# superlinear-ai/raglite

Measured on AMD Instinct MI355X. Metric: queries/sec, MaxSim 32x1M d=1024 exact top-100, higher is better.
Workload: dtype f32 in / f32 scores: candidate chunks found with the fp16 hi halves of corpus and queries (1 x v_mfma_f32_16x16x32_f16 per multiply, f32 accumulate, rigorous error bound), their scores by v_mfma_f32_16x16x4_f32 (exact f32 products); full-precision fallback: 3 x v_mfma_f32_16x16x32_f16 on hi+lo pairs

## Files before the change

### include/raglite_hip.h

```cpp
#ifndef RAGLITE_HIP_H
#define RAGLITE_HIP_H

#include <stddef.h>
#include <stdint.h>

#ifdef __cplusplus
extern "C" {
#endif

typedef enum {
    RL_OK = 0,
    RL_ERR_INVALID = -1,
    RL_ERR_HIP = -2,
    RL_ERR_UNSUPPORTED = -3,
    RL_ERR_NOMEM = -4
} rl_status;

typedef enum { RL_MEM_HOST = 0, RL_MEM_DEVICE = 1 } rl_mem;
#define RL_MEM_FILTERS_DEVICE 2
typedef enum {
    RL_ARITH_AUTO = 0,
    RL_ARITH_FP32_EXACT = 1,
    RL_ARITH_F16_SPLIT = 2,
    RL_ARITH_F16_STORED = 3
// ... 70 lines not shown
                  const float* row_sumsq, float split_scale, int32_t kernel, int32_t max_workgroups, float* out, int64_t ld,
                  float* out_q_sumsq, float* out_q_scale, int mem, void* stream);

int rl_index_create(rl_index** out, const float* embeddings, int64_t n_rows, int32_t dim,
                    const int64_t* chunk_offsets, int64_t n_chunks, int metric, int mem, void* stream);
int rl_index_create_f16(rl_index** out, const uint16_t* embeddings_f16, int64_t n_rows, int32_t dim,
                        const int64_t* chunk_offsets, int64_t n_chunks, int metric, int mem, void* stream);
int rl_index_destroy(rl_index* index);
int rl_index_info(const rl_index* index, int64_t* n_rows, int32_t* dim, int64_t* n_chunks, int* metric);
int rl_index_memory(const rl_index* index, int64_t out[8]);

#define RL_IMAGE_PRESPLIT 1u
#define RL_IMAGE_HI 2u
#define RL_IMAGE_HI_PLANE 4u
int rl_index_prepare(rl_index* index, uint32_t images, uint32_t* built, void* stream);

int rl_index_append(rl_index* index, const float* rows, int64_t n_new_rows, const int64_t* new_chunk_sizes,
                    int64_t n_new_chunks, int mem, void* stream);
int rl_index_delete_chunks(rl_index* index, const int64_t* chunk_ordinals, int64_t n, void* stream);
int rl_index_live(rl_index* index, int64_t* live_rows, int64_t* live_chunks, void* stream);
int rl_index_compact(rl_index* index, int64_t* out_remap, int64_t* new_n_rows, int64_t* new_n_chunks, void* stream);

int rl_index_set_arithmetic(rl_index* index, int mode);
int rl_index_arithmetic(rl_index* index, int* in_effect);

typedef enum {
    RL_OPT_HI_SEARCH = 1, RL_OPT_HI_MAXSIM = 2, RL_OPT_HI_PRODUCTS = 3, RL_OPT_PP_PASS = 4, RL_OPT_FUSED_TOPK = 5, RL_OPT_FUSED_HI = 6,
    RL_OPT_FUSED_PP = 7, RL_OPT_FUSED_TOPK_CAP = 8, RL_OPT_FUSED_TOPK_STRIDE = 9, RL_OPT_GEMM_PASS = 10, RL_OPT_QUERY_PAIRS = 11,
    RL_OPT_PLANES_GEMM = 12, RL_OPT_KEEP_IMAGE = 13, RL_OPT_KEEP_HI = 14, RL_OPT_IMAGE_HEADROOM_MB = 15, RL_OPT_ARITHMETIC = 16,
    RL_OPT_EXACT_KTH_THRESHOLD = 17, RL_OPT_FUSED_TWO_ROUNDS = 18, RL_OPT_KEEP_HI_PLANE = 19, RL_OPT_PAIRS_PACKED = 20,
    RL_OPT_F16_EXACT = 21, RL_OPT_LAZY_IMAGES = 22, RL_OPT_FUSED_PP_SAMPLE = 23,
    RL_OPT_LIST_SELECT = 24, RL_OPT_HI_FEW = 25, RL_OPT_TOPK_BLOCK = 26, RL_OPT_HI_PIVOT = 27, RL_OPT_COUNT_ = 28
} rl_option;
enum { RL_OPT_PP_SCHEDULE = 64, RL_OPT_PP_XCD_PASSES = 65 };
int rl_set_default_option(int key, int64_t value);
int rl_get_default_option(int key, int64_t* value);
int rl_index_set_option(rl_index* index, int key, int64_t value);
int rl_index_get_option(rl_index* index, int key, int64_t* value);

int rl_search_rows(rl_index* index, const float* queries, int32_t n_queries, int32_t k,
                   float* out_scores, int32_t* out_rows, int mem, void* stream);

int rl_rank_cut_begin(rl_index* index, const float* queries, int32_t n_queries, int mem, void* stream);
int rl_rank_cut_level(rl_index* index, int level, int64_t rank_limit, uint32_t* out_hist, int mem, void* stream);
int rl_rank_cut_level_done(rl_index* index, int level, const uint32_t* hist_sum, int mem, void* stream);
int rl_rank_cut_ties(rl_index* index, int64_t rank_limit, uint32_t* out_ties, int mem, void* stream);
int rl_rank_cut_finish(rl_index* index, int64_t rank_limit, const uint32_t* ties_before, const uint32_t* chunk_filter, int32_t k,
                       float* out_scores, int32_t* out_rows, int mem, void* stream);

int rl_search_chunks(rl_index* index, const float* queries, int32_t n_queries, int32_t num_hits,
                     int32_t k, float* out_scores, int32_t* out_chunks, int32_t* out_counts,
                     int mem, void* stream);

int rl_maxsim_topk(rl_index* index, const float* query_vecs, int32_t nq, int32_t k,
                   float* out_scores, int32_t* out_chunks, int mem, void* stream);
int rl_maxsim_scores(rl_index* index, const float* query_vecs, int32_t nq, float* out_scores,
                     int mem, void* stream);
int rl_maxsim_topk_batch(rl_index* index, const float* query_vecs, int32_t n_queries, int32_t nq, int32_t k,
                         float* out_scores, int32_t* out_chunks, int mem, void* stream);
int rl_maxsim_topk_batch_f16(rl_index* index, const uint16_t* query_vecs_f16, int32_t n_queries, int32_t nq, int32_t k,
                             float* out_scores, int32_t* out_chunks, int mem, void* stream);

int rl_maxsim_batch_begin(rl_index* index, const float* query_vecs, int32_t n_queries, int32_t nq, int32_t k, float* out_approx, int mem,
                          void* stream);
int rl_maxsim_batch_finish(rl_index* index, const float* query_vecs, const float* all_approx, int32_t world, int32_t rank, float* out_scores,
                           int32_t* out_chunks, int mem, void* stream);

// ... 181 lines not shown
```

### raglite_amd/_abi.py

```python

from __future__ import annotations

import ctypes as C
import functools
import os
from pathlib import Path

LIB_PATH = Path(os.environ.get("RAGLITE_HIP_LIB") or Path(__file__).resolve().parent / "_lib" / "libraglite_hip.so")

RL_OK, RL_ERR_INVALID, RL_ERR_HIP, RL_ERR_UNSUPPORTED, RL_ERR_NOMEM = 0, -1, -2, -3, -4
MEM_HOST, MEM_DEVICE = 0, 1
MEM_FILTERS_DEVICE = 2
METRICS = {"cosine": 0, "dot": 1, "l2": 2}
SCORE_METRICS = {"raw": 0, "cosine": 1, "dot": 2, "l2": 3}
SYNTH_KINDS = {"uniform": 0, "small_int": 1}
ATTN_DTYPES = {"bfloat16": 0, "float16": 1}
ENCODER_MAX_TOKENS = 256
ENCODER_MAX_PACK_TOKENS = 8192
ENCODER_EPILOGUES = {"bias": 0, "gelu": 1, "partial": 2}
OPTIONS = {
    "hi_search": 1, "hi_maxsim": 2, "hi_products": 3, "pp_pass": 4, "fused_topk": 5, "fused_hi": 6, "fused_pp": 7, "fused_topk_cap": 8,
    "fused_topk_stride": 9, "gemm_pass": 10, "query_pairs": 11, "planes_gemm": 12, "keep_image": 13, "keep_hi": 14,
    "image_headroom_mb": 15, "arithmetic": 16, "exact_kth_threshold": 17, "fused_two_rounds": 18,
    "keep_hi_plane": 19, "pairs_packed": 20, "f16_exact": 21, "lazy_images": 22, "fused_pp_sample": 23, "list_select": 24, "hi_few": 25, "topk_block": 26, "hi_pivot": 27,
}
SCHEDULE_OPTIONS = {"pp_schedule": 64, "pp_xcd_passes": 65}


def option_key(name: str) -> int:
    return OPTIONS[name] if name in OPTIONS else SCHEDULE_OPTIONS[name]

c_void_p, c_int, c_i32, c_i64, c_u64, c_size_t = C.c_void_p, C.c_int, C.c_int32, C.c_int64, C.c_uint64, C.c_size_t
c_double, c_char_p = C.c_double, C.c_char_p

_SIGNATURES = {
    "rl_version": [],
    "rl_last_error": [],
    "rl_init": [c_int],
    "rl_device_count": [C.POINTER(c_int)],
    "rl_device_info": [c_int, c_char_p, c_int, C.POINTER(c_int), C.POINTER(c_i64)],
    "rl_dev_alloc": [C.POINTER(c_void_p), c_size_t],
    "rl_dev_free": [c_void_p],
    "rl_memcpy_h2d": [c_void_p, c_void_p, c_size_t, c_void_p],
    "rl_memcpy_d2h": [c_void_p, c_void_p, c_size_t, c_void_p],
    "rl_memcpy_d2d": [c_void_p, c_void_p, c_size_t, c_void_p],
    "rl_stream_sync": [c_void_p],
    "rl_synth_fill": [c_void_p, c_i64, c_i64, c_u64, c_int, c_void_p],
    "rl_pool_norm": [c_void_p, c_i64, c_i32, c_void_p, c_void_p, c_i64, c_i32, c_double, c_void_p, c_void_p,
                     c_int, c_void_p],
    "rl_attention_varlen": [c_void_p, c_void_p, c_i32, c_i64, c_i32, c_i32, c_i32, c_i32, C.c_float, c_void_p, c_int, c_void_p],
    "rl_encoder_create": [C.POINTER(c_void_p), c_i32, c_i32, c_i32, c_i32, c_i32, c_i32, c_i32, C.c_float, c_i32, c_void_p, c_void_p, c_void_p,
                          c_void_p, c_void_p, c_void_p],
    "rl_encoder_forward": [c_void_p, c_void_p, c_void_p, c_void_p, c_void_p, c_i32, c_i64, c_i32, c_void_p, c_int, c_void_p],
    "rl_encoder_info": [c_void_p, c_i64, C.POINTER(c_i32), C.POINTER(c_i64), C.POINTER(c_i64), C.POINTER(c_void_p), C.POINTER(c_i32)],
    "rl_encoder_destroy": [c_void_p],
    "rl_encoder_embed": [c_void_p, c_void_p, c_void_p, c_i64, c_void_p, c_i32, c_void_p, c_i32, c_void_p, c_i32, c_void_p, c_void_p, c_i32,
                         C.c_float, c_i32, c_void_p, c_int, c_void_p],
    "rl_encoder_linear": [c_void_p, c_i64, c_i32, c_void_p, c_i32, c_void_p, c_i32, c_i32, c_void_p, c_void_p, c_int, c_void_p],
    "rl_encoder_layer_norm": [c_void_p, c_i32, c_i64, c_i32, c_void_p, c_void_p, c_void_p, c_void_p, C.c_float, c_i32, c_void_p, c_int,
# ... 192 lines not shown
```

### raglite_amd/csrc/api.hip

```cpp
#include <cmath>
#include <cstdlib>
#include <cstring>
#include <limits>
#include <memory>
#include <mutex>
#include <utility>
#include <vector>

#include "handles.h"

namespace rl {

static thread_local std::string g_last_error;
void set_error(const std::string& msg) { g_last_error = msg; }
int fail(int code, const std::string& msg) {
    g_last_error = msg;
    return code;
}

namespace {

int scan_mode(int metric) {
    switch (metric) {
        case RL_COSINE: return SCAN_COSINE;
        case RL_DOT: return SCAN_DOT;
        case RL_L2: return SCAN_L2;
        default: return -1;
    }
}

std::mutex g_default_opts_mu;
Options g_default_opts;
bool option_key_ok(int key) { return (key >= 1 && key < RL_OPT_COUNT_) || key == RL_OPT_PP_SCHEDULE || key == RL_OPT_PP_XCD_PASSES; }
bool option_value_ok(int key, int64_t value) {
    switch (key) {
        case RL_OPT_HI_SEARCH: case RL_OPT_HI_MAXSIM: case RL_OPT_PP_PASS: case RL_OPT_FUSED_TOPK: case RL_OPT_FUSED_HI: case RL_OPT_FUSED_PP:
        case RL_OPT_GEMM_PASS: case RL_OPT_QUERY_PAIRS: case RL_OPT_PLANES_GEMM: case RL_OPT_KEEP_IMAGE: case RL_OPT_KEEP_HI:
        case RL_OPT_EXACT_KTH_THRESHOLD: case RL_OPT_FUSED_TWO_ROUNDS: case RL_OPT_KEEP_HI_PLANE: case RL_OPT_F16_EXACT: case RL_OPT_LAZY_IMAGES: case RL_OPT_FUSED_PP_SAMPLE: case RL_OPT_LIST_SELECT: case RL_OPT_HI_FEW: case RL_OPT_HI_PIVOT:
        case RL_OPT_PP_SCHEDULE:
            return value == 0 || value == 1;
        case RL_OPT_PP_XCD_PASSES: return value == 8 || value == 4 || value == 2 || value == 1;
        case RL_OPT_TOPK_BLOCK: case RL_OPT_PAIRS_PACKED: return value >= 0 && value <= 2;
        case RL_OPT_HI_PRODUCTS: return value == 1 || value == 2;
        case RL_OPT_FUSED_TOPK_CAP: return value >= 0 && value <= MERGE_CAP;
        case RL_OPT_FUSED_TOPK_STRIDE: return value == 0 || (value >= 2 && value <= (int64_t(1) << 20));
        case RL_OPT_IMAGE_HEADROOM_MB: return value >= -1 && value <= (int64_t(1) << 30);
        case RL_OPT_ARITHMETIC: return value == RL_ARITH_AUTO || value == RL_ARITH_FP32_EXACT;
        default: return false;
    }
}

}

int64_t default_option(int key) {
    std::lock_guard<std::mutex> lock(g_default_opts_mu);
    return g_default_opts.v[key];
}

int use_scratch(rl_index* idx, hipStream_t s) {
    ++idx->scratch_epoch;
    idx->filt = {};
    idx->ws.block_route = (int)idx->opt.v[RL_OPT_TOPK_BLOCK];
    idx->replay.valid = false;
    return idx->last_stream.use(s);
}

}

namespace {
void update_split_scale(rl_index* idx) {
    idx->split_scale = 0.f;
    if (idx->E16 || !idx->E || idx->arithmetic == RL_ARITH_FP32_EXACT || idx->nonfinite) return;
// ... 1621 lines not shown
}

int rl_maxsim_topk(rl_index* idx, const float* query_vecs, int32_t nq, int32_t k, float* out_scores,
                   int32_t* out_chunks, int mem, void* stream) {
    return rl_maxsim_topk_filtered(idx, query_vecs, nq, k, nullptr, out_scores, out_chunks, mem, stream);
}

namespace {
struct HiBatch : HiBatchScratch {
    int32_t cap = 2048;
    bool one_product; float m_abs; const float* q_unscale;
    const float* qsum = nullptr;
    bool m_ready = true;
    bool exact_kth;
    const uint32_t* filter = nullptr;
    size_t lay(Carver c, int32_t n, int32_t k) { return HiBatchScratch::lay(c, n, k, cap, pivot_scratch_words(std::min<int32_t>(n, 2))); }
};
int hi_batch_approx(rl_index* idx, const float* d_q, int32_t nq, int32_t n_queries, int32_t n_gemm, int32_t k, float* sc, int64_t ld, HiBatch& hb,
                    hipStream_t s, bool flag_zeroed = false) {
    hb.one_product = idx->opt.v[RL_OPT_HI_PRODUCTS] == 1;
    hb.exact_kth = idx->opt.on(RL_OPT_EXACT_KTH_THRESHOLD);
    RL_TRY(carve(idx->hibuf, hb, n_gemm, k));
    const int32_t cap = hb.cap;
    hb.m_abs = idx->norm_stats.max_lo_norm + sum_eps(idx->dim) * idx->norm_stats.max_row_norm;
    QueryPlanes qp;
    qp.lay(Carver(idx->qplanes.p), n_queries, idx->dim);
    hb.q_unscale = qp.meta;
    hb.qsum = qp.qsum;
    if (!flag_zeroed) RL_HIP(hipMemsetAsync(hb.flag, 0, 16 * sizeof(uint32_t), s));
    (void)cap;
    const bool pp = hb.one_product && idx->dim >= 256 && idx->opt.on(RL_OPT_PP_PASS);
    if (pp)
        RL_TRY(launch_maxsim_pp(approx_image(idx), {idx->qplanes.p, n_queries, 0, n_gemm, nq}, chunks(idx), {sc, ld}, on(idx, s),
                                (int)idx->opt.v[RL_OPT_PP_SCHEDULE], (int)idx->opt.v[RL_OPT_PP_XCD_PASSES]));
    for (int32_t b = 0; !pp && b < n_gemm; b += GEMM_PASS_QUERIES) {
        const int32_t n_q = std::min<int32_t>(GEMM_PASS_QUERIES, n_gemm - b);
        RL_TRY(launch_maxsim_gemm(approx_image(idx), {idx->qplanes.p, n_queries, b, n_q, nq}, chunks(idx), {sc + (int64_t)b * ld, ld}, on(idx, s),
                                   hb.one_product,  false));
    }
    RL_TRY(mask_chunk_scores(idx, sc, n_gemm, ld, hb.filter, s));
    int st_pv = RL_ERR_UNSUPPORTED;
    if (n_gemm < 16 && idx->n_chunks > (int64_t)262144 && idx->opt.on(RL_OPT_HI_PIVOT))
        st_pv = launch_topk_pivot(sc, n_gemm, idx->n_chunks, ld, k, idx->ws, hb.ts, hb.ti, s);
    if (st_pv != RL_OK && st_pv != RL_ERR_UNSUPPORTED) return st_pv;
    if (st_pv == RL_ERR_UNSUPPORTED) RL_TRY(launch_topk(sc, n_gemm, idx->n_chunks, ld, k, idx->ws, hb.ts, hb.ti, s));
    return RL_OK;
}
int hi_batch_fallback(rl_index* idx, const float* d_q, int32_t nq, int32_t n_queries, int32_t n_gemm, int32_t k, float* sc, int64_t ld,
                      const HiBatch& hb, float* d_s, int32_t* d_c, hipStream_t s, bool rows_only = false);
int hi_batch_rescore(rl_index* idx, const float* d_q, int32_t nq, int32_t n_queries, int32_t n_gemm, int32_t k, float* sc, int64_t ld,
                     const HiBatch& hb, float* d_s, int32_t* d_c, hipStream_t s, bool rows_only = false) {
    const QueryVecs q{d_q, nq, (int64_t)nq * idx->dim, n_gemm};
    idx->filt = {RL_FILTER_MAXSIM_BATCH, n_gemm, hb.cap, hb.cnt, hb.flag};
    const int packed = (int)idx->opt.v[RL_OPT_PAIRS_PACKED];
    const bool m_from_qsum = !hb.m_ready && hb.qsum != nullptr;
    if (!hb.m_ready && !(hb.exact_kth && k <= hb.cap && hb.qsum)) return fail(RL_ERR_INVALID, "MaxSim batch: no bound for the candidate threshold");
    if (hb.exact_kth && k <= hb.cap) {
        RL_TRY(launch_maxsim_pairs(rows(idx), q, chunks(idx), {hb.ti, k, 0, 0, packed}, hb.es_top, s));
        if (m_from_qsum)
            RL_TRY(launch_exact_threshold(hb.es_top, hb.ti, n_gemm, k, hb.m, hb.cap, hb.thr, hb.cnt, hb.ci, hb.es, hb.flag, s, hb.qsum, hb.m_abs,
                                          idx->norm_stats.max_row_norm + idx->norm_stats.max_lo_norm, hb.one_product, hb.ts));
        else
            RL_TRY(launch_exact_threshold(hb.es_top, hb.ti, n_gemm, k, hb.m, hb.cap, hb.thr, hb.cnt, hb.ci, hb.es, hb.flag, s, nullptr, 0.f, 0.f, false, hb.ts));
        RL_TRY(launch_collect_above(sc, n_gemm, idx->n_chunks, ld, hb.thr, nullptr, hb.cap, hb.ci, nullptr, hb.cnt, hb.flag, s, hb.ts, hb.ti, k));
        if (hb.cap > k)
            RL_TRY(launch_maxsim_pairs(rows(idx), q, chunks(idx), {hb.ci, hb.cap - k, hb.cap, k, packed}, hb.es, s));
    } else {
// ... 287 lines not shown
    if (idx->live_chunk_bits) RL_TRY(launch_fix_masked(d_s, d_c, (int64_t)n_queries * k, s));
    return st.finish();
}

int rl_maxsim_approx_scores(rl_index* idx, const float* query_vecs, int32_t n_queries, int32_t nq, int kernel, float* out_scores,
                            float* out_bound, int mem, void* stream) {
    if (!idx) return fail(RL_ERR_INVALID, "rl_maxsim_approx_scores: null index");
    if (n_queries < 0 || nq < 1 || (kernel != 0 && kernel != 1)) return fail(RL_ERR_INVALID, "rl_maxsim_approx_scores: bad arguments");
    if (n_queries == 0) return RL_OK;
    if (!query_vecs || !out_scores) return fail(RL_ERR_INVALID, "rl_maxsim_approx_scores: null argument");
    hipStream_t s = as_stream(stream);
    std::lock_guard<std::mutex> lock(idx->mu);
    RL_TRY(use_scratch(idx, s));
    if (idx->has_empty_chunk || idx->n_chunks == 0)
        return fail(RL_ERR_UNSUPPORTED, "rl_maxsim_approx_scores: the approximate pass needs an index without empty chunks");
    RL_TRY(demand_images(idx, approx_image_bit(idx), s));
    if (!approx_image_valid(idx) || nq > 32 || (kernel == 0 && idx->dim < 256))
        return fail(RL_ERR_UNSUPPORTED, "rl_maxsim_approx_scores: this index keeps no HI image (or nq > 32 / dim < 256)");
    Staging st(mem, s);
    const float* d_q; float* d_o; float* d_b = nullptr;
    const size_t q_elems = (size_t)nq * idx->dim;
    const int64_t ld = idx->n_chunks;
    RL_TRY(st.in(query_vecs, (size_t)n_queries * q_elems, &d_q));
    RL_TRY(st.out(out_scores, (size_t)n_queries * ld, &d_o));
    RL_TRY(st.out(out_bound, (size_t)n_queries, &d_b));
    RL_TRY(idx->qplanes.reserve(query_planes_bytes(idx->dim, n_queries)));
    RL_TRY(launch_query_planes({d_q, nq, (int64_t)q_elems, n_queries}, idx->dim, idx->qplanes.p, s, nullptr, 0));
    const int32_t per = kernel == 0 ? n_queries : GEMM_PASS_QUERIES;
    for (int32_t b = 0; b < n_queries; b += per) {
        const QueryImageRef q{idx->qplanes.p, n_queries, b, std::min<int32_t>(per, n_queries - b), nq};
        const Scores out{d_o + (int64_t)b * ld, ld};
        if (kernel == 0)
            RL_TRY(launch_maxsim_pp(approx_image(idx), q, chunks(idx), out, on(idx, s), (int)idx->opt.v[RL_OPT_PP_SCHEDULE],
                                    (int)idx->opt.v[RL_OPT_PP_XCD_PASSES]));
        else
            RL_TRY(launch_maxsim_gemm(approx_image(idx), q, chunks(idx), out, on(idx, s),  true,  false));
    }
    if (d_b) {
        const float m_abs = idx->norm_stats.max_lo_norm + sum_eps(idx->dim) * idx->norm_stats.max_row_norm;
        QueryPlanes qp;
        qp.lay(Carver(idx->qplanes.p), n_queries, idx->dim);
        const float* q_unscale = qp.meta;
        ApproxBound L;
        RL_TRY(carve(idx->hibuf, L, n_queries));
        float *const top = L.top, *const thr = L.thr;
        uint32_t *const cnt = L.cnt, *const flag = L.flag;
        RL_HIP(hipMemsetAsync(top, 0, (size_t)n_queries * sizeof(float), s));
        RL_HIP(hipMemsetAsync(flag, 0, 16 * sizeof(uint32_t), s));
        RL_TRY(launch_maxsim_threshold(top, n_queries, 1, d_q, nq, idx->dim, (int64_t)q_elems, 1.0f, m_abs, thr, cnt, flag, s, q_unscale,
                                       idx->norm_stats.max_row_norm + idx->norm_stats.max_lo_norm));
        RL_TRY(launch_scale_f32(thr, d_b, -0.5f, n_queries, s));
        idx->filt = {};
    }
    return st.finish();
}

}

namespace rl {
int maxsim_rerank_device(rl_index* idx, const float* d_q, int32_t n_queries, int32_t nq, const int32_t* d_c, int32_t n_cand, float* d_o,
                         hipStream_t s) {
    {
        const int64_t n_items = (int64_t)n_queries * n_cand;
        RL_TRY(idx->cand.reserve((size_t)n_items * sizeof(int32_t)));
        RL_TRY(launch_sanitize_candidates(d_c, n_items, idx->n_chunks, idx->live_chunk_bits, idx->cand.as<int32_t>(), s));
        d_c = idx->cand.as<int32_t>();
    }
// ... 165 lines not shown
    else if (kind == 0 || kind == 2 || kind == 3 || kind == 5 || kind == 6) {}
    else if (kind == 9) RL_TRY(idx->scores.reserve((size_t)(idx->n_cu > 0 ? idx->n_cu : 256) * 512 * sizeof(float)));
    else if (kind == 8) {
        const auto& r = idx->replay;
        if (!r.valid || r.pools[0] != idx->misc.p || r.pools[1] != idx->fused.p || r.pools[2] != idx->pp_work.p || !hi_image_valid(idx))
            return fail(RL_ERR_UNSUPPORTED, "rl_time_kernel kind 8: no fused-HI row search ran on this index since its scratch was last resized");
    }
    else RL_TRY(idx->scores.reserve(std::max<size_t>((size_t)nq * ld * sizeof(float), 16)));
    hipEvent_t e0, e1;
    RL_HIP(hipEventCreate(&e0));
    RL_HIP(hipEventCreate(&e1));
    int st = RL_OK;
    if (kind == 2) {
        st = pairs_prepare(idx, q_dev, nq / 2, (int64_t)(nq / 2) * idx->dim, 2, s);
        if (st != RL_OK) { (void)hipEventDestroy(e0); (void)hipEventDestroy(e1); return st == RL_ERR_UNSUPPORTED ? fail(st, "rl_time_kernel: the pair kernel does not apply to this index / shape") : st; }
    }
    if (kind == 3 || kind == 5 || kind == 6) {
        st = gemm_prepare(idx, q_dev, nq / GEMM_PASS_QUERIES, (int64_t)(nq / GEMM_PASS_QUERIES) * idx->dim, GEMM_PASS_QUERIES, s, true);
        if (st == RL_OK && !image_valid(idx)) st = RL_ERR_UNSUPPORTED;
        if (st != RL_OK) { (void)hipEventDestroy(e0); (void)hipEventDestroy(e1); return st == RL_ERR_UNSUPPORTED ? fail(st, "rl_time_kernel: the eight-query kernel does not apply to this index / shape") : st; }
    }
    if (kind == 7) {
        st = pp_vec >= 1 && pp_vec * pp_n == nq ? gemm_prepare(idx, q_dev, pp_vec, (int64_t)pp_vec * idx->dim, pp_n, s) : RL_ERR_UNSUPPORTED;
        if (st == RL_OK && !(approx_image_valid(idx) && idx->dim >= 256)) st = RL_ERR_UNSUPPORTED;
        if (st != RL_OK) { (void)hipEventDestroy(e0); (void)hipEventDestroy(e1); return st == RL_ERR_UNSUPPORTED ? fail(st, "rl_time_kernel: the sixteen-query kernel does not apply to this index / shape") : st; }
    }
    if (kind == 4 || kind == 10) {
        st = demand_images(idx, IMG_HI_PLANE, s);
        if (st != RL_OK) { (void)hipEventDestroy(e0); (void)hipEventDestroy(e1); return st; }
    }
    RL_HIP(hipEventRecord(e0, s));
    for (int i = 0; i < iters && st == RL_OK; ++i) {
        if (kind == 7) st = launch_maxsim_pp(approx_image(idx), {idx->qplanes.p, pp_n, 0, pp_n, pp_vec}, chunks(idx), {idx->scores.as<float>(), ldc}, on(idx, s),
                                             (int)idx->opt.v[RL_OPT_PP_SCHEDULE], (int)idx->opt.v[RL_OPT_PP_XCD_PASSES]);
        else if (kind == 3) st = gemm_pass(idx, nq / GEMM_PASS_QUERIES, GEMM_PASS_QUERIES, 0, GEMM_PASS_QUERIES, idx->scores.as<float>(), ldc, s);
        else if (kind == 8) {
            const auto& r = idx->replay;
            const RowMetric metric = metric_of(idx, r.mode);
            if (hipMemsetAsync(r.cnt, 0, (size_t)r.B * sizeof(uint32_t), s) != hipSuccess) st = RL_ERR_HIP;
            else if (r.pp && r.round1_tiles > 0) {
                CandArgs ca1 = r.ca;
                ca1.tau = r.thr1;
                st = launch_pp_rows_pass(hi_image(idx), r.B, r.qs, metric, &ca1, {idx->pp_work.p, r.log_cap, 0, r.round1_tiles, false, r.row_test}, on(idx, s));
                if (st == RL_OK)
                    st = launch_pp_rows_pass(hi_image(idx), r.B, r.qs, metric, &r.ca, {idx->pp_work.p, r.log_cap, r.round1_tiles, -1, true, r.row_test}, on(idx, s));
            }
            else if (r.pp) st = launch_pp_rows_pass(hi_image(idx), r.B, r.qs, metric, &r.ca, {idx->pp_work.p, r.log_cap, 0, -1, false, r.row_test}, on(idx, s));
            else st = launch_score_planes_pass(hi_image(idx), r.B, r.qs, Scores{}, metric, {1, &r.ca, true}, on(idx, s));
        }
        else if (kind == 0) st = maxsim_scores_device(idx, q_dev, nq, idx->scores.as<float>(), s);
        else if (kind == 9) st = launch_mfma_f16_rate(idx->scores.as<float>(), idx->n_cu, MFMA_RATE_ITERS, s, nullptr);
        else if (kind == 2) st = pairs_pass(idx, nq / 2, 2, 0, idx->scores.as<float>(), ldc, s);
        else if (kind == 5 || kind == 6) {
            st = hi_image_valid(idx) ? launch_maxsim_gemm(hi_image(idx), {idx->qplanes.p, GEMM_PASS_QUERIES, 0, GEMM_PASS_QUERIES, nq / GEMM_PASS_QUERIES},
                                                          chunks(idx), {idx->scores.as<float>(), ldc}, on(idx, s),  kind == 6,  false)
                                     : fail(RL_ERR_UNSUPPORTED, "rl_time_kernel: the index has no HI image");
        }
        else if (kind == 4) {
            st = hi_valid(idx) ? launch_maxsim_stream(hi_plane(idx), {q_dev, nq}, chunks(idx), 1, {idx->scores.as<float>(), ld}, on(idx, s))
                               : fail(RL_ERR_UNSUPPORTED, "rl_time_kernel: the index has no HI plane");
        }
        else if (kind == 10) {
            st = hi_valid(idx) && nq <= 32 ? launch_maxsim_stream_batch(hi_plane(idx), {q_dev, nq, (int64_t)nq * idx->dim, 1}, chunks(idx),
                                                                        {idx->scores.as<float>(), ldc}, on(idx, s))
                                           : fail(RL_ERR_UNSUPPORTED, "rl_time_kernel: the index has no HI plane (or nq > 32)");
        }
        else st = score_rows(idx, q_dev, nq, ld, s);
// ... 13 lines not shown
```

### raglite_amd/csrc/common.h

```cpp
#pragma once
#include <hip/hip_runtime.h>
#include <stdint.h>

#include <algorithm>
#include <cstdlib>
#include <string>

#include "raglite_hip.h"

namespace rl {

void set_error(const std::string& msg);
int fail(int code, const std::string& msg);

#define RL_HIP(expr)                                                                         \
    do {                                                                                     \
        hipError_t _e = (expr);                                                              \
        if (_e != hipSuccess)                                                                \
            return ::rl::fail(_e == hipErrorOutOfMemory ? RL_ERR_NOMEM : RL_ERR_HIP,         \
                              std::string(#expr) + ": " + hipGetErrorString(_e));            \
    } while (0)

#define RL_TRY(expr)              \
    do {                          \
// ... 406 lines not shown
struct Launch {
    int n_cu = 0;
    hipStream_t s = nullptr;
    const uint32_t* run_if = nullptr;
};

int launch_row_to_chunk(const int64_t* chunk_offsets, int64_t n_chunks, int64_t n_rows, int32_t* row_to_chunk,
                        hipStream_t s);
int launch_maxsim_stream(const RowsRef& D, const QueryVecs& q, const ChunkMap& c, int mode, Scores out, const Launch& on);
struct StreamSecondJob {
    const float* D = nullptr;
    int64_t n_rows = 0;
    float* out = nullptr;
    int64_t ld = 0;
    const uint32_t* run_if = nullptr;
};
int launch_maxsim_stream_two(const RowsRef& D, const QueryVecs& q, const ChunkMap& c, Scores out, const Launch& on, const StreamSecondJob& job2);
int launch_maxsim_stream_batch(const RowsRef& D, const QueryVecs& q, const ChunkMap& c, Scores out, const Launch& on);
size_t query_split_bytes(int32_t dim, int32_t n_queries);
int launch_query_split(const QueryVecs& q, int32_t dim, void* buf, bool f16_corpus, hipStream_t s);
int launch_maxsim_stream2(const RowsRef& D, const QueryImageRef& q, const ChunkMap& c, Scores out, const Launch& on);
size_t planes_bytes(int64_t rows, int32_t dim, bool half = false);
int launch_presplit_rows(const RowsRef& E, int64_t first_row, void* planes, hipStream_t s);
int launch_preformat_rows16(const RowsRef& E, int64_t first_row, void* planes, hipStream_t s);
int launch_presplit_hi_rows(const RowsRef& E, int64_t first_row, void* planes, hipStream_t s);
size_t chunk_ends_words(int64_t rows);
int launch_chunk_ends(const int32_t* row_to_chunk, int64_t n_rows, uint32_t* ends, hipStream_t s);
size_t query_planes_bytes(int32_t dim, int32_t n_queries);
int launch_query_planes(const QueryVecs& q, int32_t dim, void* buf, hipStream_t s, uint32_t* zero_words, int n_zero);
int launch_maxsim_gemm(const RowsRef& image, const QueryImageRef& q, const ChunkMap& c, Scores out, const Launch& on, bool hi_only,
                       bool all_passes);
constexpr int32_t PP_PASS_QUERIES = 16;
int launch_maxsim_pp(const RowsRef& image, const QueryImageRef& q, const ChunkMap& c, Scores out, const Launch& on,
                     int schedule, int xcd_passes);
constexpr int32_t MFMA_RATE_ITERS = 1000;
int launch_mfma_f16_rate(float* out, int n_cu, int32_t iters, hipStream_t s, double* flops);
size_t score_planes_scratch_floats(int32_t nb, int32_t dim);
int launch_score_planes(const RowsRef& image, const float* Q, int32_t nb, Scores out, const RowMetric& m, float* scratch, const Launch& on);
struct CandArgs { const float* tau; int32_t tau_stride; float* scores; int32_t* ids; uint32_t* cnt; uint32_t* overflow; int32_t cap; };
int launch_score_planes_queries(const float* Q, int32_t nb, int32_t dim, float* scratch, int mode, hipStream_t s, uint32_t* zero_word = nullptr);
size_t pp_rows_scratch_bytes(int64_t n_rows, int32_t nb, int n_cu, int32_t expected_per_query, int32_t* log_cap_out);
struct PpRowsPass {
    void* work = nullptr;
    int32_t log_cap = 0;
    int64_t tile_begin = 0, tile_count = -1;
    bool norms_ready = false;
    bool row_norm_test = false;
};
int launch_pp_rows_pass(const RowsRef& image, int32_t nb, float* scratch, const RowMetric& m, const CandArgs* cand, const PpRowsPass& pass,
                        const Launch& on);
int launch_pp_rows_sample(const RowsRef& image, int32_t nb, float* scratch, const RowMetric& m, Scores S, int32_t stride, const Launch& on);
int launch_raise_threshold(float* thr, const float* kth, int32_t nq, int32_t k, const float* window, hipStream_t s);
struct ScorePass {
    int32_t tile_stride = 1;
    const CandArgs* cand = nullptr;
    bool hi_only = false;
};
int launch_score_planes_pass(const RowsRef& image, int32_t nb, float* scratch, Scores out, const RowMetric& m, const ScorePass& pass,
                             const Launch& on);
int launch_row_range(const float* E, int64_t n_rows, int32_t dim, uint32_t* range, hipStream_t s);
int launch_score_gemm(const RowsRef& E, const float* Q, int32_t nb, Scores out, const RowMetric& m, float* q_sumsq_scratch, const Launch& on,
                      int tile = 0);
int launch_query_sumsq(const float* Q, int32_t nb, int32_t dim, float* out, hipStream_t s);
size_t score_gemm_scratch_floats(int32_t nb, int32_t dim, bool split);
struct PairsList {
    const int32_t* candidates = nullptr;
    int64_t n_items = 0;
// ... 14 lines not shown
```

### raglite_amd/csrc/handles.h

```cpp
#pragma once
#include <limits>
#include <memory>
#include <mutex>
#include <vector>

#include "device_mem.h"

namespace rl {

inline int filters_mem(int mem) { return (mem & RL_MEM_FILTERS_DEVICE) ? RL_MEM_DEVICE : mem; }
inline int args_mem(int mem) { return mem & ~RL_MEM_FILTERS_DEVICE; }

constexpr size_t SCORE_BATCH_BYTES = size_t(8) << 30;

struct Options {
    int64_t v[RL_OPT_PP_XCD_PASSES + 1];
    Options() {
        for (auto& x : v) x = 0;
        v[RL_OPT_HI_SEARCH] = v[RL_OPT_HI_MAXSIM] = v[RL_OPT_HI_PRODUCTS] = v[RL_OPT_PP_PASS] = v[RL_OPT_FUSED_TOPK] = v[RL_OPT_FUSED_HI] = 1;
        v[RL_OPT_FUSED_PP] = v[RL_OPT_GEMM_PASS] = v[RL_OPT_QUERY_PAIRS] = v[RL_OPT_PLANES_GEMM] = v[RL_OPT_KEEP_IMAGE] = v[RL_OPT_KEEP_HI] = 1;
        v[RL_OPT_EXACT_KTH_THRESHOLD] = v[RL_OPT_FUSED_TWO_ROUNDS] = v[RL_OPT_KEEP_HI_PLANE] = v[RL_OPT_F16_EXACT] = v[RL_OPT_LAZY_IMAGES] = v[RL_OPT_FUSED_PP_SAMPLE] = v[RL_OPT_LIST_SELECT] = v[RL_OPT_HI_FEW] = 1;
        v[RL_OPT_TOPK_BLOCK] = v[RL_OPT_PAIRS_PACKED] = 2;
        v[RL_OPT_HI_PIVOT] = 1;
        v[RL_OPT_PP_SCHEDULE] = 1;
        v[RL_OPT_PP_XCD_PASSES] = 2;
        v[RL_OPT_IMAGE_HEADROOM_MB] = -1;
        v[RL_OPT_ARITHMETIC] = RL_ARITH_AUTO;
    }
    bool on(int key) const { return v[key] != 0; }
};

struct Image {
    Pool buf;
    float scale = 0.f;
    int64_t rows = 0;
    void drop() {
        buf.release();
        scale = 0.f;
        rows = 0;
    }
    bool covers(float at, int64_t n_rows) const { return scale > 0.f && scale == at && rows == n_rows && n_rows > 0; }
};
struct NormStats {
    float max_row_norm = 0.f, max_lo_norm = 0.f, max_lo_ratio = 0.f;
    float min_row_norm = std::numeric_limits<float>::infinity();
    float max_row_norm_scale = 0.f;
    int64_t max_row_norm_rows = 0;
    void reset() { *this = NormStats(); }
    bool measured(int64_t n_rows) const { return max_row_norm_rows == n_rows && max_row_norm > 0.f; }
};

struct LastStream {
    hipStream_t stream = nullptr;
    bool set = false;
    int use(hipStream_t s) {
        if (set && stream != s) RL_HIP(hipStreamSynchronize(stream));
        stream = s;
        set = true;
// ... 148 lines not shown
```

### raglite_amd/csrc/maxsim_pp.hip

```cpp
#include <cstdio>
#include <cstdlib>
#include <utility>

#include "common.h"
#include "pp_schedule.h"
#include "scratch_layout.h"

namespace rl {

typedef float f32x4 __attribute__((ext_vector_type(4)));
typedef _Float16 h16x8 __attribute__((ext_vector_type(8)));

namespace {
constexpr int PP_RT = 128;
constexpr int PP_NBLK = PP_RT / 16;
constexpr int PP_QPP = 16;
constexpr int PP_DC = 8;
constexpr int PP_LC = 6;
constexpr int PP_CSLOT = PP_NBLK * 1024;
constexpr int PP_STAGE = 1536;
constexpr int PP_LDS = PP_DC * PP_CSLOT + 16 * PP_STAGE * 4;

__device__ __forceinline__ int64_t pp_uniform_i64(int64_t v) {
    const uint32_t lo = __builtin_amdgcn_readfirstlane((uint32_t)(uint64_t)v);
// ... 30 lines not shown
    f32x16s v;
    const float* const u = reinterpret_cast<const float*>(pp_uniform_i64(reinterpret_cast<int64_t>(p)));
    asm volatile("s_load_dwordx16 %0, %1, 0x0\n\ts_waitcnt lgkmcnt(0)" : "=s"(v) : "s"(u) : "memory");
    return v;
}
__device__ __forceinline__ h16x8 pp_h(const f32x4& v) {
    h16x8 r;
    __builtin_memcpy(&r, &v, 16);
    return r;
}
}

struct PpRows {
    const float* tau;
    const float* q_unscale;
    const float* q_sumsq;
    const float* row_norm;
    const float* blk_minmax;
    int32_t B, QT, metric;
    float* cand_scores; int32_t* cand_ids; uint32_t* cand_cnt; uint32_t* overflow; int32_t cap;
    uint2* log; int32_t log_cap;
    int32_t tile_begin, tile_count;
    float* S; int64_t ld_s; int32_t stride;
    int32_t xcd_passes, dma_hint;
};

template <int DBG, int MODE, bool ROWNORM>
__global__ __launch_bounds__(512, 2) void maxsim_pp_kernel(const char* __restrict__ planes, int64_t n_rows, int32_t nslab,
                                                           const char* __restrict__ qfrag, const float* __restrict__ qmeta, int32_t n_q,
                                                           const int32_t* __restrict__ row_to_chunk, const int64_t* __restrict__ chunk_offsets,
                                                           const uint32_t* __restrict__ ends_bits, float* __restrict__ out, int64_t out_stride,
                                                           float inv_e_scale, const uint32_t* __restrict__ run_if, PpRows rs) {
    constexpr bool ROWS = MODE == 2, SCORES = MODE == 1, GROUPS = ROWS || SCORES;
    constexpr bool TILES = MODE == 3;
    static_assert(!TILES || DBG == 0, "the timing skeletons keep the slab-counting loop");
    __shared__ __attribute__((aligned(16))) char smem[PP_LDS];
    if (run_if && __builtin_amdgcn_readfirstlane((int)*run_if) == 0) return;
    const int lane = threadIdx.x & 63;
    const int wv = wave_id();
    int64_t G = gridDim.x, b = blockIdx.x;
    int qt = (int)blockIdx.y;
    if constexpr (!GROUPS) {
        const int32_t passes = (n_q + PP_QPP - 1) / PP_QPP;
        const PpSlot m = gridDim.y > 1 ? pp_schedule((int32_t)blockIdx.x, (int32_t)blockIdx.y, (int32_t)gridDim.x, (int32_t)gridDim.y, passes)
                                       : pp_schedule_affine((int32_t)blockIdx.x, (int32_t)gridDim.x, passes, rs.xcd_passes);
        G = __builtin_amdgcn_readfirstlane(m.ranges);
        b = __builtin_amdgcn_readfirstlane(m.range);
        qt = __builtin_amdgcn_readfirstlane(m.pass);
    }
    auto boundary = [&](int64_t t) -> int64_t {
        if (t <= 0) return 0;
        if (t >= n_rows) return n_rows;
        const int32_t c = row_to_chunk[t];
        const int64_t c0 = chunk_offsets[c], c1 = chunk_offsets[c + 1];
        return c0 == t ? t : c1;
    };
    int32_t r_lo = 0, r_hi = 0, nt_rows = 0;
    if constexpr (!GROUPS) {
        r_lo = (int32_t)pp_uniform_i64(boundary((n_rows * b) / G));
        r_hi = (int32_t)pp_uniform_i64((b + 1 == G) ? n_rows : boundary((n_rows * (b + 1)) / G));
        if (r_hi <= r_lo) return;
    } else {
        const int64_t Tr = rs.tile_count;
        const int64_t t0 = (Tr * b) / G, t1 = (Tr * (b + 1)) / G;
        nt_rows = (int32_t)(t1 - t0);
        if (nt_rows <= 0) return;
        r_lo = (int32_t)((rs.tile_begin + t0) * PP_RT);
        r_hi = (int32_t)n_rows;
// ... 518 lines not shown
    auto main_loop = [&](auto LAG_) __attribute__((always_inline)) {
        if constexpr (TILES) {
            const int pairs = nslab >> 1;
            prologue_fragments();
            for (int t = 0; t < nt; ++t) {
                pp_tile_ends(t);
                slab(qA, qB, LAG_, std::true_type{});
                landed(qB);
                slab(qB, qA, LAG_, std::false_type{});
                landed(qA);
#pragma nounroll
                for (int p = 1; p < pairs; ++p) {
                    slab(qA, qB, LAG_, std::false_type{});
                    landed(qB);
                    slab(qB, qA, LAG_, std::false_type{});
                    landed(qA);
                }
                asm volatile("s_waitcnt lgkmcnt(0)" : "+s"(tile_ends) : : "memory");
                [&]<int... A>(std::integer_sequence<int, A...>) { (block_epilogue_maxsim(std::integral_constant<int, A>{}, t), ...); }
                (std::make_integer_sequence<int, PP_NBLK>{});
                if (own_cnt - own_flushed > PP_STAGE - PP_RT) flush_out();
            }
        } else {
            for (int g = 0; g < total; g += 2) {
                slab(qA, qB, LAG_, std::false_type{});
                landed(qB);
                if (g + 1 < total) {
                    slab(qB, qA, LAG_, std::false_type{});
                    landed(qA);
                }
            }
        }
    };
#undef PP_I
    if (wv < 4) main_loop(std::false_type{});
    else main_loop(std::true_type{});
    asm volatile("s_waitcnt vmcnt(0)" ::: "memory");
    dump_log();
    flush_rows();
    flush_out();
    if constexpr (DBG & 128) {
        if (n_q > 1000000) {
            f32x4 t = (f32x4){0.f, 0.f, 0.f, 0.f};
#pragma unroll
            for (int q = 0; q < 2; ++q)
#pragma unroll
                for (int qb = 0; qb < 2; ++qb)
#pragma unroll
                    for (int a = 0; a < PP_NBLK; ++a) t += acc[q][qb][a];
            out[lane] = (t[0] + t[1]) + (t[2] + t[3]);
        }
    }
}

int launch_maxsim_pp(const RowsRef& rows, const QueryImageRef& q, const ChunkMap& c, Scores o, const Launch& on, int schedule, int xcd_passes) {
    const auto [image, one_plane, n_rows, dim, split_scale] = rows;
    const auto [qbuf, n_queries, first, n_q, nq] = q;
    const auto [row_to_chunk, chunk_offsets, n_chunks, ends_bits] = c;
    const auto [out, out_stride] = o;
    const auto [n_cu, s, run_if] = on;
    if (!one_plane) return RL_ERR_UNSUPPORTED;
    if (nq < 1 || nq > 32 || n_q < 1 || n_q > PP_QPP * 4096 || n_rows < 1 || first < 0 || first + n_q > n_queries) return RL_ERR_UNSUPPORTED;
    if (dim % 32 || dim < 256 || !(split_scale > 0.f) || !image || !ends_bits) return RL_ERR_UNSUPPORTED;
    const int32_t nslab = dim / 32;
    const char* qfrag = static_cast<const char*>(qbuf) + (size_t)first * nslab * 4096;
    QueryPlanes L;
    L.lay(Carver(const_cast<void*>(qbuf)), n_queries, dim);
    const float* qmeta = L.meta + 2 * (size_t)first;
    const int64_t tiles = (n_rows + PP_RT - 1) / PP_RT;
    const int64_t gx = std::max<int64_t>(1, std::min<int64_t>(n_cu > 0 ? n_cu : 256, tiles)), passes = (n_q + PP_QPP - 1) / PP_QPP;
    const dim3 grid = schedule == 1 ? dim3((unsigned)(gx * passes)) : dim3((unsigned)gx, (unsigned)passes), blk(512);
    PpRows rs{};
    rs.xcd_passes = schedule == 1 ? xcd_passes : 8;
#define RL_PP_LAUNCH(DBG_) RL_PP_LAUNCH_MODE(DBG_, 0)
#define RL_PP_LAUNCH_MODE(DBG_, MODE_)                                                                                                     \
    hipLaunchKernelGGL((maxsim_pp_kernel<DBG_, MODE_, false>), grid, blk, 0, s, static_cast<const char*>(image), n_rows, nslab, qfrag, qmeta, n_q, row_to_chunk, \
                       chunk_offsets, ends_bits, out, out_stride, 1.0f / split_scale, run_if, rs)
#ifdef RAGLITE_EXPERIMENTS
    const int force_hint = std::getenv("RAGLITE_PP_HINT") ? std::atoi(std::getenv("RAGLITE_PP_HINT")) : -1;
    if (force_hint >= PP_HINT_NONE && force_hint <= PP_HINT_SC1) rs.dma_hint = force_hint;
    const int dbg = std::getenv("RAGLITE_PP_DBG") ? std::atoi(std::getenv("RAGLITE_PP_DBG")) : 0;
    if (dbg == 2) RL_PP_LAUNCH(2);
    else if (dbg == 128) RL_PP_LAUNCH(128);
    else if (dbg == 136) RL_PP_LAUNCH(136);
    else if (dbg == 144) RL_PP_LAUNCH(144);
    else if (dbg == 160) RL_PP_LAUNCH(160);
    else if (dbg == 184) RL_PP_LAUNCH(184);
    else if (dbg == 1 || nslab % 2) RL_PP_LAUNCH(0);
    else RL_PP_LAUNCH_MODE(0, 3);
#else
    if (nslab % 2) RL_PP_LAUNCH(0);
    else RL_PP_LAUNCH_MODE(0, 3);
#endif
#undef RL_PP_LAUNCH
#undef RL_PP_LAUNCH_MODE
    RL_HIP(hipGetLastError());
    return RL_OK;
}

__global__ __launch_bounds__(256) void block_norm_minmax_kernel(const float* __restrict__ row_norm, int64_t n_rows, int64_t n_blocks,
                                                                 float* __restrict__ out) {
    const int64_t blk = (int64_t)blockIdx.x * 256 + threadIdx.x;
    if (blk >= n_blocks) return;
    float mn = INFINITY, mx = 0.f;
    for (int i = 0; i < 16; ++i) {
        const int64_t r = blk * 16 + i;
        if (r < n_rows) { const float v = row_norm[r]; mn = fminf(mn, v); mx = fmaxf(mx, v); }
    }
    out[2 * blk] = mn;
    out[2 * blk + 1] = mx;
}

int launch_pp_rows_sample(const RowsRef& rows, int32_t nb, float* scratch, const RowMetric& m, Scores out, int32_t stride, const Launch& on) {
    const auto [image, one_plane, n_rows, dim, split_scale] = rows;
    const auto [mode, row_norm, row_sumsq] = m;
    const auto [S, ld_s] = out;
    const auto [n_cu, s, run_if] = on;
    if (!one_plane || run_if) return RL_ERR_UNSUPPORTED;
    if (nb < 1 || n_rows < 1 || dim % 32 || dim < 256 || !(split_scale > 0.f) || !image || !S || stride < 1) return RL_ERR_UNSUPPORTED;
    if (mode != SCAN_COSINE && mode != SCAN_DOT) return RL_ERR_UNSUPPORTED;
    if (mode == SCAN_COSINE && !row_norm) return RL_ERR_INVALID;
    if ((ld_s & 255) || (reinterpret_cast<uintptr_t>(S) & 15)) return RL_ERR_UNSUPPORTED;
    const int32_t nslab = dim / 32, groups = (nb + 31) / 32;
    ScoreQueries L;
// ... 130 lines not shown
```

Baseline: 18940.

## Add alternating double-buffered query-register main loop for MaxSim PP kernel

Adds a new kernel mode (MODE 4) with an alternating main loop. Two query register sets (qA/qB) are ping-ponged so the next slab's query and corpus loads are issued while MFMAs run on the current set. Explicit s_barrier, waitcnt and sched_barrier placement replaces the split-by-wave main_loop, and the tile epilogue is interleaved around barriers. A new pp_loop option, on by default, selects it, at the cost of more live registers and hand-tuned synchronisation that could stall or raise register pressure.

```diff
diff --git a/include/raglite_hip.h b/include/raglite_hip.h
--- a/include/raglite_hip.h
+++ b/include/raglite_hip.h
@@ -126,7 +126,7 @@
     RL_OPT_F16_EXACT = 21, RL_OPT_LAZY_IMAGES = 22, RL_OPT_FUSED_PP_SAMPLE = 23,
     RL_OPT_LIST_SELECT = 24, RL_OPT_HI_FEW = 25, RL_OPT_TOPK_BLOCK = 26, RL_OPT_HI_PIVOT = 27, RL_OPT_COUNT_ = 28
 } rl_option;
-enum { RL_OPT_PP_SCHEDULE = 64, RL_OPT_PP_XCD_PASSES = 65 };
+enum { RL_OPT_PP_SCHEDULE = 64, RL_OPT_PP_XCD_PASSES = 65, RL_OPT_PP_LOOP = 66 };
 int rl_set_default_option(int key, int64_t value);
 int rl_get_default_option(int key, int64_t* value);
 int rl_index_set_option(rl_index* index, int key, int64_t value);
diff --git a/raglite_amd/_abi.py b/raglite_amd/_abi.py
--- a/raglite_amd/_abi.py
+++ b/raglite_amd/_abi.py
@@ -24,7 +24,7 @@
     "image_headroom_mb": 15, "arithmetic": 16, "exact_kth_threshold": 17, "fused_two_rounds": 18,
     "keep_hi_plane": 19, "pairs_packed": 20, "f16_exact": 21, "lazy_images": 22, "fused_pp_sample": 23, "list_select": 24, "hi_few": 25, "topk_block": 26, "hi_pivot": 27,
 }
-SCHEDULE_OPTIONS = {"pp_schedule": 64, "pp_xcd_passes": 65}
+SCHEDULE_OPTIONS = {"pp_schedule": 64, "pp_xcd_passes": 65, "pp_loop": 66}
 
 
 def option_key(name: str) -> int:
diff --git a/raglite_amd/csrc/api.hip b/raglite_amd/csrc/api.hip
--- a/raglite_amd/csrc/api.hip
+++ b/raglite_amd/csrc/api.hip
@@ -31,13 +31,13 @@
 
 std::mutex g_default_opts_mu;
 Options g_default_opts;
-bool option_key_ok(int key) { return (key >= 1 && key < RL_OPT_COUNT_) || key == RL_OPT_PP_SCHEDULE || key == RL_OPT_PP_XCD_PASSES; }
+bool option_key_ok(int key) { return (key >= 1 && key < RL_OPT_COUNT_) || key == RL_OPT_PP_SCHEDULE || key == RL_OPT_PP_XCD_PASSES || key == RL_OPT_PP_LOOP; }
 bool option_value_ok(int key, int64_t value) {
     switch (key) {
         case RL_OPT_HI_SEARCH: case RL_OPT_HI_MAXSIM: case RL_OPT_PP_PASS: case RL_OPT_FUSED_TOPK: case RL_OPT_FUSED_HI: case RL_OPT_FUSED_PP:
         case RL_OPT_GEMM_PASS: case RL_OPT_QUERY_PAIRS: case RL_OPT_PLANES_GEMM: case RL_OPT_KEEP_IMAGE: case RL_OPT_KEEP_HI:
         case RL_OPT_EXACT_KTH_THRESHOLD: case RL_OPT_FUSED_TWO_ROUNDS: case RL_OPT_KEEP_HI_PLANE: case RL_OPT_F16_EXACT: case RL_OPT_LAZY_IMAGES: case RL_OPT_FUSED_PP_SAMPLE: case RL_OPT_LIST_SELECT: case RL_OPT_HI_FEW: case RL_OPT_HI_PIVOT:
-        case RL_OPT_PP_SCHEDULE:
+        case RL_OPT_PP_SCHEDULE: case RL_OPT_PP_LOOP:
             return value == 0 || value == 1;
         case RL_OPT_PP_XCD_PASSES: return value == 8 || value == 4 || value == 2 || value == 1;
         case RL_OPT_TOPK_BLOCK: case RL_OPT_PAIRS_PACKED: return value >= 0 && value <= 2;
@@ -1725,7 +1725,7 @@
     const bool pp = hb.one_product && idx->dim >= 256 && idx->opt.on(RL_OPT_PP_PASS);
     if (pp)
         RL_TRY(launch_maxsim_pp(approx_image(idx), {idx->qplanes.p, n_queries, 0, n_gemm, nq}, chunks(idx), {sc, ld}, on(idx, s),
-                                (int)idx->opt.v[RL_OPT_PP_SCHEDULE], (int)idx->opt.v[RL_OPT_PP_XCD_PASSES]));
+                                (int)idx->opt.v[RL_OPT_PP_SCHEDULE], (int)idx->opt.v[RL_OPT_PP_XCD_PASSES], (int)idx->opt.v[RL_OPT_PP_LOOP]));
     for (int32_t b = 0; !pp && b < n_gemm; b += GEMM_PASS_QUERIES) {
         const int32_t n_q = std::min<int32_t>(GEMM_PASS_QUERIES, n_gemm - b);
         RL_TRY(launch_maxsim_gemm(approx_image(idx), {idx->qplanes.p, n_queries, b, n_q, nq}, chunks(idx), {sc + (int64_t)b * ld, ld}, on(idx, s),
@@ -2079,7 +2079,7 @@
         const Scores out{d_o + (int64_t)b * ld, ld};
         if (kernel == 0)
             RL_TRY(launch_maxsim_pp(approx_image(idx), q, chunks(idx), out, on(idx, s), (int)idx->opt.v[RL_OPT_PP_SCHEDULE],
-                                    (int)idx->opt.v[RL_OPT_PP_XCD_PASSES]));
+                                    (int)idx->opt.v[RL_OPT_PP_XCD_PASSES], (int)idx->opt.v[RL_OPT_PP_LOOP]));
         else
             RL_TRY(launch_maxsim_gemm(approx_image(idx), q, chunks(idx), out, on(idx, s),  true,  false));
     }
@@ -2311,7 +2311,7 @@
     RL_HIP(hipEventRecord(e0, s));
     for (int i = 0; i < iters && st == RL_OK; ++i) {
         if (kind == 7) st = launch_maxsim_pp(approx_image(idx), {idx->qplanes.p, pp_n, 0, pp_n, pp_vec}, chunks(idx), {idx->scores.as<float>(), ldc}, on(idx, s),
-                                             (int)idx->opt.v[RL_OPT_PP_SCHEDULE], (int)idx->opt.v[RL_OPT_PP_XCD_PASSES]);
+                                             (int)idx->opt.v[RL_OPT_PP_SCHEDULE], (int)idx->opt.v[RL_OPT_PP_XCD_PASSES], (int)idx->opt.v[RL_OPT_PP_LOOP]);
         else if (kind == 3) st = gemm_pass(idx, nq / GEMM_PASS_QUERIES, GEMM_PASS_QUERIES, 0, GEMM_PASS_QUERIES, idx->scores.as<float>(), ldc, s);
         else if (kind == 8) {
             const auto& r = idx->replay;
diff --git a/raglite_amd/csrc/common.h b/raglite_amd/csrc/common.h
--- a/raglite_amd/csrc/common.h
+++ b/raglite_amd/csrc/common.h
@@ -462,7 +462,7 @@
                        bool all_passes);
 constexpr int32_t PP_PASS_QUERIES = 16;
 int launch_maxsim_pp(const RowsRef& image, const QueryImageRef& q, const ChunkMap& c, Scores out, const Launch& on,
-                     int schedule, int xcd_passes);
+                     int schedule, int xcd_passes, int loop);
 constexpr int32_t MFMA_RATE_ITERS = 1000;
 int launch_mfma_f16_rate(float* out, int n_cu, int32_t iters, hipStream_t s, double* flops);
 size_t score_planes_scratch_floats(int32_t nb, int32_t dim);
diff --git a/raglite_amd/csrc/handles.h b/raglite_amd/csrc/handles.h
--- a/raglite_amd/csrc/handles.h
+++ b/raglite_amd/csrc/handles.h
@@ -14,7 +14,7 @@
 constexpr size_t SCORE_BATCH_BYTES = size_t(8) << 30;
 
 struct Options {
-    int64_t v[RL_OPT_PP_XCD_PASSES + 1];
+    int64_t v[RL_OPT_PP_LOOP + 1];
     Options() {
         for (auto& x : v) x = 0;
         v[RL_OPT_HI_SEARCH] = v[RL_OPT_HI_MAXSIM] = v[RL_OPT_HI_PRODUCTS] = v[RL_OPT_PP_PASS] = v[RL_OPT_FUSED_TOPK] = v[RL_OPT_FUSED_HI] = 1;
@@ -24,6 +24,7 @@
         v[RL_OPT_HI_PIVOT] = 1;
         v[RL_OPT_PP_SCHEDULE] = 1;
         v[RL_OPT_PP_XCD_PASSES] = 2;
+        v[RL_OPT_PP_LOOP] = 1;
         v[RL_OPT_IMAGE_HEADROOM_MB] = -1;
         v[RL_OPT_ARITHMETIC] = RL_ARITH_AUTO;
     }
diff --git a/raglite_amd/csrc/maxsim_pp.hip b/raglite_amd/csrc/maxsim_pp.hip
--- a/raglite_amd/csrc/maxsim_pp.hip
+++ b/raglite_amd/csrc/maxsim_pp.hip
@@ -86,8 +86,9 @@
                                                            const uint32_t* __restrict__ ends_bits, float* __restrict__ out, int64_t out_stride,
                                                            float inv_e_scale, const uint32_t* __restrict__ run_if, PpRows rs) {
     constexpr bool ROWS = MODE == 2, SCORES = MODE == 1, GROUPS = ROWS || SCORES;
-    constexpr bool TILES = MODE == 3;
-    static_assert(!TILES || DBG == 0, "the timing skeletons keep the slab-counting loop");
+    constexpr bool ALT = MODE == 4;
+    constexpr bool TILES = MODE == 3 || ALT;
+    static_assert(!TILES || DBG == 0 || (ALT && DBG == 128), "the timing skeletons keep the slab-counting loop (but the bare alternating loop)");
     __shared__ __attribute__((aligned(16))) char smem[PP_LDS];
     if (run_if && __builtin_amdgcn_readfirstlane((int)*run_if) == 0) return;
     const int lane = threadIdx.x & 63;
@@ -672,8 +673,87 @@
             }
         }
     };
+    [[maybe_unused]] auto alt_mfmas = [&](f32x4 (&q)[4], auto FIRST_) __attribute__((always_inline)) {
+        __builtin_amdgcn_sched_barrier(0);
+        [&]<int... A>(std::integer_sequence<int, A...>) { (mfma_group(q, std::integral_constant<int, A>{}, FIRST_), ...); }
+        (std::make_integer_sequence<int, PP_NBLK>{});
+        __builtin_amdgcn_sched_barrier(0);
+    };
+    [[maybe_unused]] auto alt_barrier = [&]() __attribute__((always_inline)) {
+        asm volatile("s_barrier" ::: "memory");
+        __builtin_amdgcn_sched_barrier(0);
+    };
+    [[maybe_unused]] auto alt_compute = [&](f32x4 (&q)[4], auto FIRST_) __attribute__((always_inline)) {
+        alt_mfmas(q, FIRST_);
+        alt_barrier();
+    };
+    [[maybe_unused]] auto alt_issue = [&](f32x4 (&qn)[4]) __attribute__((always_inline)) {
+        issue_qregs(qn);
+        issue_c();
+        [&]<int... A>(std::integer_sequence<int, A...>) { (read_slab(std::integral_constant<int, A>{}), ...); }
+        (std::make_integer_sequence<int, PP_NBLK>{});
+        c_slot = c_slot + 1 == PP_DC ? 0 : c_slot + 1;
+        __builtin_amdgcn_sched_barrier(0);
+    };
+    [[maybe_unused]] auto alt_wait = [&](f32x4 (&qc)[4]) __attribute__((always_inline)) {
+        __builtin_amdgcn_sched_barrier(0);
+        asm volatile("s_waitcnt lgkmcnt(0)" ::: "memory");
+        asm volatile("s_waitcnt vmcnt(6)" ::: "memory");
+        pp_pin(ef[0], ef[1], ef[2], ef[3]);
+        pp_pin(ef[4], ef[5], ef[6], ef[7]);
+        pp_pin(qc[0], qc[1], qc[2], qc[3]);
+        __builtin_amdgcn_sched_barrier(0);
+    };
+    [[maybe_unused]] auto alt_landed = [&](f32x4 (&qc)[4]) __attribute__((always_inline)) {
+        alt_wait(qc);
+        alt_barrier();
+    };
+    [[maybe_unused]] auto alt_loop = [&]() __attribute__((always_inline)) {
+        const int pairs = nslab >> 1;
+        issue_c();
+        issue_qregs(qA);
+        issue_qregs(qB);
+        asm volatile("s_waitcnt vmcnt(0)\n\ts_barrier" ::: "memory");
+        [&]<int... A>(std::integer_sequence<int, A...>) { (read_slab(std::integral_constant<int, A>{}), ...); }
+        (std::make_integer_sequence<int, PP_NBLK>{});
+        c_slot = 1;
+        asm volatile("s_waitcnt lgkmcnt(0)" ::: "memory");
+        pp_pin(ef[0], ef[1], ef[2], ef[3]);
+        pp_pin(ef[4], ef[5], ef[6], ef[7]);
+        pp_pin(qA[0], qA[1], qA[2], qA[3]);
+        pp_pin(qB[0], qB[1], qB[2], qB[3]);
+        if (wv >= 4) asm volatile("s_barrier" ::: "memory");
+        for (int t = 0; t < nt; ++t) {
+            if constexpr (!(DBG & 128)) pp_tile_ends(t);
+            alt_compute(qA, std::true_type{});
+#pragma nounroll
+            for (int p = 1; p < pairs; ++p) {
+                alt_issue(qA); alt_landed(qB);
+                alt_compute(qB, std::false_type{});
+                alt_issue(qB); alt_landed(qA);
+                alt_compute(qA, std::false_type{});
+            }
+            alt_issue(qA); alt_landed(qB);
+            alt_mfmas(qB, std::false_type{});
+            if (wv < 4) alt_barrier();
+            alt_issue(qB);
+            if constexpr (!(DBG & 128)) {
+                asm volatile("" : "+s"(tile_ends));
+                [&]<int... A>(std::integer_sequence<int, A...>) { (block_epilogue_maxsim(std::integral_constant<int, A>{}, t), ...); }
+                (std::make_integer_sequence<int, PP_NBLK - 1>{});
+            }
+            if (wv >= 4) alt_barrier();
+            if constexpr (!(DBG & 128)) {
+                block_epilogue_maxsim(std::integral_constant<int, PP_NBLK - 1>{}, t);
+                if (own_cnt - own_flushed > PP_STAGE - PP_RT) flush_out();
+            }
+            alt_landed(qA);
+        }
+        if (wv < 4) asm volatile("s_barrier" ::: "memory");
+    };
 #undef PP_I
-    if (wv < 4) main_loop(std::false_type{});
+    if constexpr (ALT) alt_loop();
+    else if (wv < 4) main_loop(std::false_type{});
     else main_loop(std::true_type{});
     asm volatile("s_waitcnt vmcnt(0)" ::: "memory");
     dump_log();
@@ -693,7 +773,8 @@
     }
 }
 
-int launch_maxsim_pp(const RowsRef& rows, const QueryImageRef& q, const ChunkMap& c, Scores o, const Launch& on, int schedule, int xcd_passes) {
+int launch_maxsim_pp(const RowsRef& rows, const QueryImageRef& q, const ChunkMap& c, Scores o, const Launch& on, int schedule, int xcd_passes,
+                     int loop) {
     const auto [image, one_plane, n_rows, dim, split_scale] = rows;
     const auto [qbuf, n_queries, first, n_q, nq] = q;
     const auto [row_to_chunk, chunk_offsets, n_chunks, ends_bits] = c;
@@ -726,10 +807,13 @@
     else if (dbg == 144) RL_PP_LAUNCH(144);
     else if (dbg == 160) RL_PP_LAUNCH(160);
     else if (dbg == 184) RL_PP_LAUNCH(184);
+    else if (dbg == 132 && nslab % 2 == 0) RL_PP_LAUNCH_MODE(128, 4);
     else if (dbg == 1 || nslab % 2) RL_PP_LAUNCH(0);
+    else if (loop == 1) RL_PP_LAUNCH_MODE(0, 4);
     else RL_PP_LAUNCH_MODE(0, 3);
 #else
     if (nslab % 2) RL_PP_LAUNCH(0);
+    else if (loop == 1) RL_PP_LAUNCH_MODE(0, 4);
     else RL_PP_LAUNCH_MODE(0, 3);
 #endif
 #undef RL_PP_LAUNCH
```

Result: faster. 19700, median of 6 (+4.0%).
